# adolfogonzalez3/custom_envs

Measured on AMD Instinct MI355X. Metric: vectorised env-steps/sec, Optimize-v0 @4096 envs, 1/2/4/8 MI355X vs host CPU, higher is better.
Workload: dtype f64; 1 GPU; Optimize-v0 softmax-regression 256x10 (P=20, obs 41), 4096 envs per GPU, B=N=256, 40-step episodes with in-kernel auto-reset, device-resident actions/outputs; envs_per_gpu=4096, global_envs=4096, n_rows=256, n_features=10, n_classes=2, batch_size=256, steps_per_launch=250, outputs=every step kept: a [250]-record slab per launch, parallelism=env-sharded x1 (no collective)

## Files before the change

custom_envs_amd/csrc/optimize_lr_persist.h:

```cpp
#pragma once

#include "optimize_lr_mfma.h"

namespace ce {

struct ManyArgs {
    int k;
    long long act_stride;
    long long out_step;
};

constexpr int kLpWaves = 4;
constexpr int kLpMaxTpw = 8;

#ifndef CE_LP_G4
#define CE_LP_G4 1
#endif
#ifndef CE_LP_G4_XF
#define CE_LP_G4_XF 1
#endif
#ifndef CE_LP_EPI_SLEEP
#define CE_LP_EPI_SLEEP 0
#endif
#ifndef CE_LP_ROW_PRIO
#define CE_LP_ROW_PRIO 3
#endif
#ifndef CE_LP_LOG_HEAD
#define CE_LP_LOG_HEAD 1
#endif
#ifndef CE_LP_WD_HANDOVER
#define CE_LP_WD_HANDOVER 1
#endif
#ifndef CE_LP_GA_REGS
#define CE_LP_GA_REGS 4
#endif
__host__ __device__ constexpr bool lp_g4(int nkf) { return CE_LP_G4 && nkf <= 3; }
constexpr int kLpWdWave = 2;
constexpr int kLpWdRing = 2;

__host__ __device__ constexpr int lp_tpw(int N, int W = kLpWaves) {
    const int per = ((N + 15) / 16 + W - 1) / W;
    return per <= 1 ? 1 : per <= 2 ? 2 : per <= 4 ? 4 : per <= 8 ? 8 : 0;
}
__host__ __device__ constexpr bool lp_pad(int N, int W = kLpWaves) {
    return N % 16 != 0 || (N + 15) / 16 != W * lp_tpw(N, W);
}

#ifdef CE_DIAG
#define LP_STAMP(k)                                                   \
    do {                                                              \
        __builtin_amdgcn_sched_barrier(0);                            \
        lp_st[k] = __builtin_amdgcn_s_memrealtime();                  \
        __builtin_amdgcn_sched_barrier(0);                            \
    } while (0)
#else
#define LP_STAMP(k) \
    do {            \
    } while (0)
#endif

template <int NKF, int TPW, bool PAD, int W>
__global__ __launch_bounds__(kWave * W) void optimize_lr_persist_kernel(StepArgs<double> a, ManyArgs m) {
    constexpr int BLK = kWave * W;
    constexpr int P_MAX = 2 * kLrMaxF;
    constexpr int TD = lr_tile_doubles(NKF);
    constexpr int PR = (kLrEnvs * P_MAX + BLK - 1) / BLK;
    constexpr int OSM = 2 * P_MAX + 4;
    constexpr int NG = TPW < 4 ? TPW : 4;
    __shared__ double red_s[2][W][4][kWave];
    __shared__ double red_l[2][W][kLrEnvs];
    __shared__ double red_h[2][W][kLrEnvs];
    __shared__ __attribute__((aligned(16))) float obs_s[2][kLrEnvs * OSM];
    __shared__ double tab_s[CE_LR_TEXP ? kLrExpTab : 1];

#ifdef CE_DIAG
    unsigned long long lp_st[8] = {0};
#endif
    LP_STAMP(0);
    const int tid = threadIdx.x;
    const int lane = tid & (kWave - 1);
    const int wave = __builtin_amdgcn_readfirstlane(tid >> 6);
    const int c = lane & 15, h = lane >> 4;
    const int E = a.E, F = a.F, P = 2 * F, N = a.N, B = a.B;
    const int OS = a.obs_stride, OL = a.obs_lo;
    const int e0 = blockIdx.x * kLrEnvs;
    const int e = e0 + c;
    const bool env_ok = e < E;
    const unsigned pbase = static_cast<unsigned>(env_ok ? e : 0) * P;
    const double *img = reinterpret_cast<const double *>(a.data);
    const int ntiles = (N + 15) / 16;

#if CE_LR_TEXP
    LrExpSlice<BLK> tslice;
    tslice.load(img + static_cast<unsigned>(ntiles) * TD + kLrMaxF, tid);
#endif
    unsigned ioff[NKF];
    double2 wv[NKF], w0v[NKF];
    float2 av[NKF];
#if CE_LR_NOCLAMP
    double xm[NKF];
    const double *colmax = img + static_cast<unsigned>(ntiles) * TD;
#endif
#pragma unroll
    for (int k = 0; k < NKF; ++k) {
        const int f = 4 * k + h;
        ioff[k] = pbase + (f < F ? 2 * f : 0);
        wv[k] = *reinterpret_cast<const double2 *>(a.W + ioff[k]);
        w0v[k] = *reinterpret_cast<const double2 *>(a.W0 + ioff[k]);
        av[k] = *reinterpret_cast<const float2 *>(a.act + ioff[k]);
#if CE_LR_NOCLAMP
        xm[k] = colmax[f];
#endif
    }
    double xf[TPW][NKF], xg[TPW][4];
    unsigned vmask = 0;
#pragma unroll
    for (int i = 0; i < TPW; ++i) {
        const int t = wave + W * i;
        const bool live = !PAD || t < ntiles;
        const double *ti = img + static_cast<unsigned>(live ? t : 0) * TD;
#pragma unroll
        for (int k = 0; k < NKF; ++k) xf[i][k] = live ? ti[k * kWave + lane] : 0.0;
#pragma unroll
        for (int q = 0; q < 4; ++q) xg[i][q] = live ? ti[(NKF + q) * kWave + lane] : 0.0;
        if constexpr (PAD) {
            const int2 ya = reinterpret_cast<const int2 *>(ti + (NKF + 4) * kWave)[lane];
            const int2 yb = reinterpret_cast<const int2 *>(ti + (NKF + 5) * kWave)[lane];
            const int ys[4] = {ya.x, ya.y, yb.x, yb.y};
#pragma unroll
            for (int q = 0; q < 4; ++q) vmask |= (live && ys[q] >= 0 ? 1u : 0u) << (4 * i + q);
        }
    }
    int step_c = a.step[env_ok ? e : 0];
    const int np_ = kLrEnvs * P;
    const int pmul = (65536 + P - 1) / P;
    int pj[PR], pp[PR], step_p[PR];
    bool prole[PR];
    unsigned gi[PR];
    double g_prev[PR], rG[PR];
#pragma unroll
    for (int r = 0; r < PR; ++r) {
        const int i = tid + r * BLK;
        pj[r] = (i * pmul) >> 16;
        pp[r] = i - pj[r] * P;
        prole[r] = i < np_ && e0 + pj[r] < E;
        gi[r] = static_cast<unsigned>(prole[r] ? e0 + pj[r] : 0) * P + (prole[r] ? pp[r] : 0);
        g_prev[r] = a.G[gi[r]];
        step_p[r] = a.step[prole[r] ? e0 + pj[r] : 0];
    }
    const int sj = tid - (BLK - kLrEnvs);
    const bool srole = sj >= 0 && e0 + sj < E;
    const unsigned es = srole ? e0 + sj : 0;
    double lprev = a.L[es];
    int step_s = a.step[es];
#if CE_LR_TEXP
    tslice.store(tab_s, tid);
    __syncthreads();
#endif
    const double dB = static_cast<double>(B), rB = a.inv_B;
    double rL = rcp_newton2(lprev + 0.1);
#pragma unroll
    for (int r = 0; r < PR; ++r) rG[r] = rcp_newton2(fabs(g_prev[r]) + 1.0);
    if (OL == 0)
        for (int i = tid; i < kLrEnvs * OS; i += BLK) {
            const int j = i / OS, p = i - j * OS;
            if (p < P) obs_s[0][i] = obs_s[1][i] = 0.0f;
        }

    double wd[NKF];
    auto margins = [&]() {
#pragma unroll
        for (int k = 0; k < NKF; ++k) {
            const int f = 4 * k + h;
            const double w0 = wv[k].x - static_cast<double>(av[k].x);
            const double w1 = wv[k].y - static_cast<double>(av[k].y);
            wv[k] = double2{w0, w1};
            wd[k] = f < F ? w0 - w1 : 0.0;
        }
    };
    margins();
#ifdef CE_DIAG
    asm volatile("s_waitcnt vmcnt(0)" ::: "memory");
#endif
    LP_STAMP(1);

    constexpr int QC = 4;
    auto forward = [&](const double (&xv)[NKF]) {
        lr_d4 u = {0.0, 0.0, 0.0, 0.0};
#pragma unroll
        for (int k = 0; k < NKF; ++k) u = __builtin_amdgcn_mfma_f64_16x16x4f64(xv[k], wd[k], u, 0, 0, 0);
        return u;
    };
    const int nenv = E - e0 < kLrEnvs ? E - e0 : kLrEnvs;
    auto flush_obs = [&](int t) {
        float *ob = reinterpret_cast<float *>(reinterpret_cast<char *>(a.obs) + t * m.out_step) +
                    static_cast<unsigned>(e0) * OS;
        const float *src = obs_s[t & 1];
        const int nfl = nenv * OS, n4 = nfl >> 2;
        for (int i = tid; i < n4; i += BLK) {
            typedef float lp_f4 __attribute__((ext_vector_type(4)));
            const lp_f4 v = *reinterpret_cast<const lp_f4 *>(&src[4 * i]);
            asm volatile("global_store_dwordx4 %0, %1, off sc1" ::"v"(ob + 4 * i), "v"(v) : "memory");
        }
        for (int i = 4 * n4 + tid; i < nfl; i += BLK) lr_store(&ob[i], src[i]);
    };

    for (int t = 0; t < m.k; ++t) {
        const int buf = t & 1;
        float2 an[NKF];
        {
            const float *actn = a.act + (t + 1 < m.k ? (t + 1) * m.act_stride : 0);
#pragma unroll
            for (int k = 0; k < NKF; ++k) an[k] = *reinterpret_cast<const float2 *>(actn + ioff[k]);
        }
#if CE_LR_NOCLAMP
        double ub = 0.0;
#pragma unroll
        for (int k = 0; k < NKF; ++k) ub = fma(fabs(wd[k]), xm[k], ub);
        const int tier = lr_tier(ub);
#else
        const int tier = kLrClamped;
#endif
        lr_d4 sacc = {0.0, 0.0, 0.0, 0.0};
        double prod = 1.0, nlog = 0.0, umin = 1.0;
        unsigned miss = 0;
        auto rows = [&](auto tier_c) {
            constexpr int TIER = decltype(tier_c)::value;
#pragma unroll
            for (int g0 = 0; g0 < TPW; g0 += NG) {
                if (g0 > 0) {
                    nlog -= lr_log(prod, tab_s);
                    prod = 1.0;
                }
                lr_d4 u[NG];
#pragma unroll
                for (int i = 0; i < NG; ++i) u[i] = forward(xf[g0 + i]);
#pragma unroll
                for (int i = 0; i < NG; ++i) {
                    double qv[4];
                    static_assert(QC == 4, "the tile's four values go through the exp together");
                    double tx[QC];
                    bool valid[QC];
#pragma unroll
                    for (int j = 0; j < QC; ++j) {
                        if constexpr (TIER == kLrClamped) tx[j] = clamp_u(u[i][j]);
                        else tx[j] = u[i][j];
                        valid[j] = !PAD || ((vmask >> (4 * (g0 + i) + j)) & 1u);
                    }
                    lr_exp_neg<QC>(tx, tab_s);
                    if constexpr (TIER == kLrBatched) {
                        lr_post4(u[i], tx, valid, qv, prod, miss);
                    } else {
#pragma unroll
                        for (int j = 0; j < QC; ++j) lr_post(u[i][j], tx[j], valid[j], qv[j], prod, miss);
                    }
                    lr_tie4<TIER>(u[i], valid, umin);
#pragma unroll
                    for (int q = 0; q < 4; ++q)
                        sacc = __builtin_amdgcn_mfma_f64_16x16x4f64(xg[g0 + i][q], qv[q], sacc, 0, 0, 0);
                }
            }
        };
        lr_run_tier(tier, rows);
        int hits = 4 * TPW - lr_miss_count(miss);
        if (__any(umin < 0x1p-52)) {
#pragma unroll
            for (int i = 0; i < TPW; ++i) {
                const int tt = wave + W * i;
                if (tt >= ntiles) continue;
                const double *ti = img + static_cast<unsigned>(tt) * TD;
                const int2 ya = reinterpret_cast<const int2 *>(ti + (NKF + 4) * kWave)[lane];
                const int2 yb = reinterpret_cast<const int2 *>(ti + (NKF + 5) * kWave)[lane];
                const int yv[4] = {ya.x, ya.y, yb.x, yb.y};
                const lr_d4 uu = forward(xf[i]);
                double tx[4];
#pragma unroll
                for (int q = 0; q < 4; ++q) tx[q] = abs_clamp750(uu[q]);
                exp_neg_multi_clamped<4>(tx);
#pragma unroll
                for (int q = 0; q < 4; ++q)
                    if (yv[q] >= 0 && tx[q] == 1.0) hits += (yv[q] == 0 ? 1 : 0) - lr_hit(uu[q]);
            }
        }
        double lsum = nlog - lr_log(prod, tab_s);
        lsum = fold_pair<16>(lsum, lsum);
        lsum = fold_pair<32>(lsum, lsum);
        const double hsum = static_cast<double>(fold_env_lanes(hits));
#pragma unroll
        for (int r = 0; r < 4; ++r) red_s[buf][wave][r][lane] = sacc[r];
        if (lane < kLrEnvs) {
            red_l[buf][wave][lane] = lsum;
            red_h[buf][wave][lane] = hsum;
        }
        {
            const bool wipe = step_c + 1 >= a.max_steps && a.auto_reset;
            step_c = wipe ? 0 : step_c + 1;
#pragma unroll
            for (int k = 0; k < NKF; ++k)
                if (wipe) wv[k] = w0v[k];
            if (t + 1 < m.k) {
#pragma unroll
                for (int k = 0; k < NKF; ++k) av[k] = an[k];
                margins();
            }
        }
        __syncthreads();
#ifdef CE_DIAG
        if (t == 0) LP_STAMP(2);
        if (t == 1) LP_STAMP(3);
        if (t == m.k - 1) LP_STAMP(4);
#endif
        if (t > 0) flush_obs(t - 1);

        const long long ro = t * m.out_step;
        if (srole) {
            double lt = 0.0, ht = 0.0;
#pragma unroll
            for (int w = 0; w < W; ++w) {
                lt += red_l[buf][w][sj];
                ht += red_h[buf][w][sj];
            }
            const double loss = div_rcp(lt, dB, rB);
            const double acc = div_rcp(ht, dB, rB);
            const double lnew = div_rcp(loss - lprev, lprev + 0.1, rL);
            const int cur = step_s + 1;
            const bool wipe = cur >= a.max_steps && a.auto_reset;
            if (a.reward) lr_store(reinterpret_cast<float *>(reinterpret_cast<char *>(a.reward) + ro) + es,
                                   static_cast<float>(-loss));
            lr_store(reinterpret_cast<float *>(reinterpret_cast<char *>(a.objective) + ro) + es,
                     static_cast<float>(loss));
            lr_store(reinterpret_cast<float *>(reinterpret_cast<char *>(a.accuracy) + ro) + es,
                     static_cast<float>(acc));
            if (a.done) (reinterpret_cast<uint8_t *>(a.done) + ro)[es] = cur >= a.max_steps ? 1 : 0;
            lr_store(reinterpret_cast<int32_t *>(reinterpret_cast<char *>(a.episode_len) + ro) + es, cur);
            obs_s[buf][sj * OS + P - OL] = wipe ? 0.0f : static_cast<float>(lnew);
            lprev = wipe ? 0.0 : lnew;
            step_s = wipe ? 0 : cur;
            rL = rcp_newton2(lprev + 0.1);
        }
#pragma unroll
        for (int r = 0; r < PR; ++r) {
            if (!prole[r]) continue;
            const bool wipe = step_p[r] + 1 >= a.max_steps && a.auto_reset;
            const int f = pp[r] >> 1;
            double sf = 0.0;
#pragma unroll
            for (int w = 0; w < W; ++w) sf += red_s[buf][w][f >> 2][pj[r] + 16 * (f & 3)];
            const double g = div_rcp((pp[r] & 1) ? sf : -sf, dB, rB);
            const double gnew = div_rcp(g, fabs(g_prev[r]) + 1.0, rG[r]);
            obs_s[buf][pj[r] * OS + P + 1 + pp[r] - OL] = wipe ? 0.0f : static_cast<float>(gnew);
            g_prev[r] = wipe ? 0.0 : gnew;
            step_p[r] = wipe ? 0 : step_p[r] + 1;
            rG[r] = rcp_newton2(fabs(g_prev[r]) + 1.0);
        }
    }
    LP_STAMP(5);
    __syncthreads();
    if (m.k > 0) flush_obs(m.k - 1);
    if (wave == 0 && env_ok) {
#pragma unroll
        for (int k = 0; k < NKF; ++k)
            if (4 * k + h < F) {
                lr_store(a.W + ioff[k], wv[k].x);
                lr_store(a.W + ioff[k] + 1, wv[k].y);
            }
    }
#pragma unroll
    for (int r = 0; r < PR; ++r)
        if (prole[r]) lr_store(&a.G[gi[r]], g_prev[r]);
    if (srole) {
        lr_store(&a.L[es], lprev);
        lr_store(&a.step[es], step_s);
    }
#ifdef CE_DIAG
    asm volatile("s_waitcnt vmcnt(0)" ::: "memory");
    LP_STAMP(6);
    const int row = blockIdx.x * W + wave;
    if (row < E && lane < 8) a.diag[static_cast<size_t>(row) * 8 + lane] = lp_st[lane];
#endif
}


template <int NKF, int TPW, bool PAD>
__global__ __launch_bounds__(512) void optimize_lr_persist_ws_kernel(
    double *Wp, const float *actp, const unsigned char *datap, double *Gp, int32_t *stepp, double *Lp,
    unsigned efp, int Np, StepArgs<double> a, ManyArgs m) {
    constexpr int W = 4;
    constexpr int BLK = 512;
    constexpr int EB = BLK - kWave * W;
    constexpr int P_MAX = 2 * kLrMaxF;
    constexpr int TD = lr_tile_doubles(NKF);
    constexpr int PR = (kLrEnvs * P_MAX + EB - 1) / EB;
    constexpr int OSM = 2 * P_MAX + 4;
    constexpr int NG = TPW < 4 ? TPW : 4;
    __shared__ double red_s[2][W][4][kWave];
    __shared__ double red_l[2][W][kLrEnvs];
    __shared__ double red_h[2][W][kLrEnvs];
    __shared__ __attribute__((aligned(16))) float obs_s[2][kLrEnvs * OSM];
    constexpr bool G4 = lp_g4(NKF);
    constexpr int G4S = 14;
    constexpr int NR = CE_LP_GA_REGS < TPW ? CE_LP_GA_REGS : TPW;
    constexpr int GS0 = G4 && NR > 0 ? 1 - NR : -NR;
    constexpr int NGS = TPW + GS0 > 0 ? TPW + GS0 : 1;
    __shared__ __attribute__((aligned(16))) double xgs[G4 ? 1 : W][G4 ? 1 : NGS][4][kWave];
    __shared__ __attribute__((aligned(16))) double xga[G4 ? W : 1][G4 ? NGS : 1][16][G4S];
    __shared__ double tab_s[CE_LR_TEXP ? kLrExpTab : 1];
#if CE_LP_WD_HANDOVER
    __shared__ double wd_s[kLpWdRing][NKF][kWave];
    __shared__ int tier_s[kLpWdRing];
#endif

#ifdef CE_DIAG
    unsigned long long lp_st[8] = {0};
#endif
    LP_STAMP(0);
    const int tid = threadIdx.x;
    const int lane = tid & (kWave - 1);
    const int wave = __builtin_amdgcn_readfirstlane(tid >> 6);
    const int c = lane & 15, h = lane >> 4;
    const int E = static_cast<int>(efp & 0xffffffu), F = static_cast<int>(efp >> 24), P = 2 * F, N = Np, B = a.B;
    const int OS = a.obs_stride, OL = a.obs_lo;
    const int e0 = blockIdx.x * kLrEnvs;
    const double *img = reinterpret_cast<const double *>(datap);
    const int ntiles = (N + 15) / 16;
    const int nenv = E - e0 < kLrEnvs ? E - e0 : kLrEnvs;

#if CE_LR_TEXP
    LrExpSlice<BLK> tslice;
    tslice.load(img + static_cast<unsigned>(ntiles) * TD + kLrMaxF, tid);
#endif
    if (wave < W) {
#if CE_LP_ROW_PRIO > 0
        __builtin_amdgcn_s_setprio(CE_LP_ROW_PRIO);
#endif
#if !CE_LP_WD_HANDOVER
        const int e = e0 + c;
        const bool env_ok = e < E;
        const unsigned pbase = static_cast<unsigned>(env_ok ? e : 0) * P;
        unsigned ioff[NKF];
        double2 wv[NKF], w0v[NKF];
        float2 av[NKF];
#if CE_LR_NOCLAMP
        double xm[NKF];
        const double *colmax = img + static_cast<unsigned>(ntiles) * TD;
#endif
#pragma unroll
        for (int k = 0; k < NKF; ++k) {
            const int f = 4 * k + h;
            ioff[k] = pbase + (f < F ? 2 * f : 0);
            wv[k] = *reinterpret_cast<const double2 *>(Wp + ioff[k]);
            av[k] = *reinterpret_cast<const float2 *>(actp + ioff[k]);
#if CE_LR_NOCLAMP
            xm[k] = colmax[f];
#endif
        }
#endif
        double xf[TPW][NKF];
#if !CE_LP_WD_HANDOVER
#pragma unroll
        for (int k = 0; k < NKF; ++k) w0v[k] = *reinterpret_cast<const double2 *>(a.W0 + ioff[k]);
#endif
        [[maybe_unused]] double gvr[NR > 0 ? NR : 1][G4 ? 4 * NKF : 4];
        unsigned vmask = 0;
#pragma unroll
        for (int i = 0; i < TPW; ++i) {
            const int t = wave + W * i;
            const bool live = !PAD || t < ntiles;
            const double *ti = img + static_cast<unsigned>(live ? t : 0) * TD;
#pragma unroll
            for (int k = 0; k < NKF; ++k) xf[i][k] = live ? ti[k * kWave + lane] : 0.0;
            if constexpr (G4) {
                const int s = i < NR ? 0 : i + GS0;
#if CE_LP_G4_XF
                const int km = 4 * (c & 3) + h, j4 = c >> 2;
#pragma unroll
                for (int g = 0; g < NKF; ++g)
                    if (i >= NR) xga[wave][s][km][j4 * NKF + g] = xf[i][g];
#else
                const int b4 = (lane >> 2) & 3, km = 4 * (lane >> 4) + (lane & 3);
#pragma unroll
                for (int q = 0; q < 4; ++q)
                    if (i >= NR && b4 < NKF) xga[wave][s][km][q * NKF + b4] = live ? ti[(NKF + q) * kWave + lane] : 0.0;
#endif
            } else if (i >= NR) {
#pragma unroll
                for (int q = 0; q < 4; ++q)
                    xgs[wave][i + GS0][q][lane] = live ? ti[(NKF + q) * kWave + lane] : 0.0;
            } else {
#pragma unroll
                for (int q = 0; q < 4; ++q) gvr[i][q] = live ? ti[(NKF + q) * kWave + lane] : 0.0;
            }
            if constexpr (PAD) {
                const int2 ya = reinterpret_cast<const int2 *>(ti + (NKF + 4) * kWave)[lane];
                const int2 yb = reinterpret_cast<const int2 *>(ti + (NKF + 5) * kWave)[lane];
                const int ys[4] = {ya.x, ya.y, yb.x, yb.y};
#pragma unroll
                for (int q = 0; q < 4; ++q) vmask |= (live && ys[q] >= 0 ? 1u : 0u) << (4 * i + q);
            }
        }
        if constexpr (G4 && NR > 0) {
            typedef double lp_d2 __attribute__((ext_vector_type(2)));
            const lp_d2 *src = reinterpret_cast<const lp_d2 *>(&xga[wave][0][4 * (lane >> 4) + (lane & 3)][0]);
#pragma unroll
            for (int i = 0; i < NR; ++i) {
#if CE_LP_G4_XF
                const int km = 4 * (c & 3) + h, j4 = c >> 2;
#pragma unroll
                for (int g = 0; g < NKF; ++g) xga[wave][0][km][j4 * NKF + g] = xf[i][g];
#else
                const int t = wave + W * i;
                const bool live = !PAD || t < ntiles;
                const double *ti = img + static_cast<unsigned>(live ? t : 0) * TD;
                const int b4 = (lane >> 2) & 3, km = 4 * (lane >> 4) + (lane & 3);
#pragma unroll
                for (int q = 0; q < 4; ++q)
                    if (b4 < NKF) xga[wave][0][km][q * NKF + b4] = live ? ti[(NKF + q) * kWave + lane] : 0.0;
#endif
                __builtin_amdgcn_wave_barrier();
#pragma unroll
                for (int p2 = 0; p2 < 2 * NKF; ++p2) {
                    const lp_d2 v = src[p2];
                    gvr[i][2 * p2] = v.x;
                    gvr[i][2 * p2 + 1] = v.y;
                }
                __builtin_amdgcn_wave_barrier();
            }
        }
#if !CE_LP_WD_HANDOVER
        int step_c = stepp[env_ok ? e : 0];
#endif
#if CE_LR_TEXP
        tslice.store(tab_s, tid);
#endif
#if CE_LR_TEXP || CE_LP_WD_HANDOVER
        __syncthreads();
#endif
        double wd[NKF];
#if CE_LP_WD_HANDOVER
        int slot = 0;
#else
        auto margins = [&]() {
#pragma unroll
            for (int k = 0; k < NKF; ++k) {
                const int f = 4 * k + h;
                const double w0 = wv[k].x - static_cast<double>(av[k].x);
                const double w1 = wv[k].y - static_cast<double>(av[k].y);
                wv[k] = double2{w0, w1};
                wd[k] = f < F ? w0 - w1 : 0.0;
            }
        };
        margins();
#endif
#ifdef CE_DIAG
        asm volatile("s_waitcnt vmcnt(0)" ::: "memory");
#endif
        LP_STAMP(1);
        constexpr int QC = 4;
        auto forward = [&](const double (&xv)[NKF]) {
            lr_d4 u = {0.0, 0.0, 0.0, 0.0};
#pragma unroll
            for (int k = 0; k < NKF; ++k) u = __builtin_amdgcn_mfma_f64_16x16x4f64(xv[k], wd[k], u, 0, 0, 0);
            return u;
        };
        for (int t = 0; t < m.k; ++t) {
            const int buf = t & 1;
#if CE_LP_WD_HANDOVER
#pragma unroll
            for (int k = 0; k < NKF; ++k) wd[k] = wd_s[slot][k][lane];
#if CE_LR_NOCLAMP
            const int tier = __builtin_amdgcn_readfirstlane(tier_s[slot]);
#else
            const int tier = kLrClamped;
#endif
            slot = slot == kLpWdRing - 1 ? 0 : slot + 1;
#else
            float2 an[NKF];
            {
                const float *actn = actp + (t + 1 < m.k ? (t + 1) * m.act_stride : 0);
#pragma unroll
                for (int k = 0; k < NKF; ++k) an[k] = *reinterpret_cast<const float2 *>(actn + ioff[k]);
            }
#if CE_LR_NOCLAMP
            double ub = 0.0;
#pragma unroll
            for (int k = 0; k < NKF; ++k) ub = fma(fabs(wd[k]), xm[k], ub);
            const int tier = lr_tier(ub);
#else
            const int tier = kLrClamped;
#endif
#endif
            lr_d4 sacc = {0.0, 0.0, 0.0, 0.0};
            double gacc[NKF];
#pragma unroll
            for (int g = 0; g < NKF; ++g) gacc[g] = 0.0;
            double prod = 1.0, nlog = 0.0, umin = 1.0;
            unsigned miss = 0;
            [[maybe_unused]] LrLogHead lhead = {};
            auto rows = [&](auto tier_c) {
                constexpr int TIER = decltype(tier_c)::value;
#pragma unroll
                for (int g0 = 0; g0 < TPW; g0 += NG) {
                    if (g0 > 0) {
                        nlog -= lr_log(prod, tab_s);
                        prod = 1.0;
                    }
                    lr_d4 u[NG];
#pragma unroll
                    for (int i = 0; i < NG; ++i) u[i] = forward(xf[g0 + i]);
#pragma unroll
                    for (int i = 0; i < NG; ++i) {
                        double gv[G4 ? 4 * NKF : 4];
                        if (g0 + i < NR) {
#pragma unroll
                            for (int j = 0; j < (G4 ? 4 * NKF : 4); ++j) gv[j] = gvr[g0 + i < NR ? g0 + i : 0][j];
                        } else if constexpr (G4) {
                            typedef double lp_d2 __attribute__((ext_vector_type(2)));
                            const lp_d2 *src = reinterpret_cast<const lp_d2 *>(
                                &xga[wave][g0 + i + GS0][4 * (lane >> 4) + (lane & 3)][0]);
#pragma unroll
                            for (int p2 = 0; p2 < 2 * NKF; ++p2) {
                                const lp_d2 v = src[p2];
                                gv[2 * p2] = v.x;
                                gv[2 * p2 + 1] = v.y;
                            }
                        } else {
#pragma unroll
                            for (int q = 0; q < 4; ++q) gv[q] = xgs[wave][g0 + i + GS0][q][lane];
                        }
                        double qv[4];
                        static_assert(QC == 4, "the tile's four values go through the exp together");
                        double tx[QC];
                        bool valid[QC];
#pragma unroll
                        for (int j = 0; j < QC; ++j) {
                            if constexpr (TIER == kLrClamped) tx[j] = clamp_u(u[i][j]);
                            else tx[j] = u[i][j];
                            valid[j] = !PAD || ((vmask >> (4 * (g0 + i) + j)) & 1u);
                        }
                        lr_exp_neg<QC>(tx, tab_s);
                        if constexpr (TIER == kLrBatched) {
                            lr_post4(u[i], tx, valid, qv, prod, miss);
                        } else {
#pragma unroll
                            for (int j = 0; j < QC; ++j)
                                lr_post(u[i][j], tx[j], valid[j], qv[j], prod, miss);
                        }
                        lr_tie4<TIER>(u[i], valid, umin);
#if CE_LP_LOG_HEAD
                        if (g0 + NG >= TPW && i == NG - 1) {
                            lhead = lr_log_head(prod, tab_s);
                            __builtin_amdgcn_sched_barrier(0);
                        }
#endif
                        if constexpr (G4) {
#pragma unroll
                            for (int q = 0; q < 4; ++q)
#pragma unroll
                                for (int g = 0; g < NKF; ++g)
                                    gacc[g] = __builtin_amdgcn_mfma_f64_4x4x4f64(gv[q * NKF + g], qv[q], gacc[g], 0, 0, 0);
                        } else {
#pragma unroll
                            for (int q = 0; q < 4; ++q)
                                sacc = __builtin_amdgcn_mfma_f64_16x16x4f64(gv[q], qv[q], sacc, 0, 0, 0);
                        }
                    }
                }
            };
            lr_run_tier(tier, rows);
            int hits = 4 * TPW - lr_miss_count(miss);
            if (__any(umin < 0x1p-52)) {
#pragma unroll
                for (int i = 0; i < TPW; ++i) {
                    const int tt = wave + W * i;
                    if (tt >= ntiles) continue;
                    const double *ti = img + static_cast<unsigned>(tt) * TD;
                    const int2 ya = reinterpret_cast<const int2 *>(ti + (NKF + 4) * kWave)[lane];
                    const int2 yb = reinterpret_cast<const int2 *>(ti + (NKF + 5) * kWave)[lane];
                    const int yv[4] = {ya.x, ya.y, yb.x, yb.y};
                    const lr_d4 uu = forward(xf[i]);
                    double tx[4];
#pragma unroll
                    for (int q = 0; q < 4; ++q) tx[q] = abs_clamp750(uu[q]);
                    exp_neg_multi_clamped<4>(tx);
#pragma unroll
                    for (int q = 0; q < 4; ++q)
                        if (yv[q] >= 0 && tx[q] == 1.0) hits += (yv[q] == 0 ? 1 : 0) - lr_hit(uu[q]);
                }
            }
#if CE_LP_LOG_HEAD
            double lsum = nlog - lr_log_tail(lhead);
#else
            double lsum = nlog - lr_log(prod, tab_s);
#endif
            lsum = fold_pair<16>(lsum, lsum);
            lsum = fold_pair<32>(lsum, lsum);
            const double hsum = static_cast<double>(fold_env_lanes(hits));
            if constexpr (G4) {
#pragma unroll
                for (int g = 0; g < NKF; ++g) red_s[buf][wave][g][lane] = gacc[g];
            } else {
#pragma unroll
                for (int r = 0; r < 4; ++r) red_s[buf][wave][r][lane] = sacc[r];
            }
            if (lane < kLrEnvs) {
                red_l[buf][wave][lane] = lsum;
                red_h[buf][wave][lane] = hsum;
            }
#if !CE_LP_WD_HANDOVER
            {
                const bool wipe = step_c + 1 >= a.max_steps && a.auto_reset;
                step_c = wipe ? 0 : step_c + 1;
                if (__any(wipe)) {
#pragma unroll
                    for (int k = 0; k < NKF; ++k)
                        if (wipe) wv[k] = w0v[k];
                }
                if (t + 1 < m.k) {
#pragma unroll
                    for (int k = 0; k < NKF; ++k) av[k] = an[k];
                    margins();
                }
            }
#endif
#ifdef CE_DIAG
            if (t == 1) LP_STAMP(7);
#endif
            __syncthreads();
#ifdef CE_DIAG
            if (t == 0) LP_STAMP(2);
            if (t == 1) LP_STAMP(3);
            if (t == m.k - 1) LP_STAMP(4);
#endif
        }
        LP_STAMP(5);
        __syncthreads();
#if !CE_LP_WD_HANDOVER
        if (wave == 0 && env_ok) {
#pragma unroll
            for (int k = 0; k < NKF; ++k)
                if (4 * k + h < F) {
                    lr_store(Wp + ioff[k], wv[k].x);
                    lr_store(Wp + ioff[k] + 1, wv[k].y);
                }
        }
#endif
    } else {
        const int te = tid - kWave * W;
        const int np_ = kLrEnvs * P;
        const int pmul = (65536 + P - 1) / P;
        int pj[PR], pp[PR], step_p[PR];
        bool prole[PR];
        unsigned gi[PR];
        double g_prev[PR], rG[PR];
#pragma unroll
        for (int r = 0; r < PR; ++r) {
            const int i = te + r * EB;
            pj[r] = (i * pmul) >> 16;
            pp[r] = i - pj[r] * P;
            prole[r] = i < np_ && e0 + pj[r] < E;
            gi[r] = static_cast<unsigned>(prole[r] ? e0 + pj[r] : 0) * P + (prole[r] ? pp[r] : 0);
            g_prev[r] = Gp[gi[r]];
            step_p[r] = stepp[prole[r] ? e0 + pj[r] : 0];
        }
        const int sj = te - (EB - kLrEnvs);
        const bool srole = sj >= 0 && e0 + sj < E;
        const unsigned es = srole ? e0 + sj : 0;
        double lprev = Lp[es];
        int step_s = stepp[es];
#if CE_LP_WD_HANDOVER
        const bool wown = wave == W + kLpWdWave;
        const int e = e0 + c;
        const bool env_ok = e < E;
        unsigned ioff[NKF];
        double2 wv[NKF], w0v[NKF];
        float2 an[NKF];
        [[maybe_unused]] double xm[NKF];
        int step_c = 0;
        auto wd_wipe = [&]() {
            const bool wipe = step_c + 1 >= a.max_steps && a.auto_reset;
            step_c = wipe ? 0 : step_c + 1;
            if (__any(wipe)) {
#pragma unroll
                for (int k = 0; k < NKF; ++k)
                    if (wipe) wv[k] = w0v[k];
            }
        };
        auto wd_emit = [&](int slot, const float2 (&av)[NKF]) {
            double wd[NKF];
#pragma unroll
            for (int k = 0; k < NKF; ++k) {
                const int f = 4 * k + h;
                const double w0 = wv[k].x - static_cast<double>(av[k].x);
                const double w1 = wv[k].y - static_cast<double>(av[k].y);
                wv[k] = double2{w0, w1};
                wd[k] = f < F ? w0 - w1 : 0.0;
            }
#if CE_LR_NOCLAMP
            double ub = 0.0;
#pragma unroll
            for (int k = 0; k < NKF; ++k) ub = fma(fabs(wd[k]), xm[k], ub);
            tier_s[slot] = lr_tier(ub);
#endif
#pragma unroll
            for (int k = 0; k < NKF; ++k) wd_s[slot][k][lane] = wd[k];
        };
        auto act_load = [&](int s, float2 (&av)[NKF]) {
            const float *acts = actp + s * m.act_stride;
#pragma unroll
            for (int k = 0; k < NKF; ++k) av[k] = *reinterpret_cast<const float2 *>(acts + ioff[k]);
        };
        if (wown) {
            const unsigned pbase = static_cast<unsigned>(env_ok ? e : 0) * P;
#if CE_LR_NOCLAMP
            const double *colmax = img + static_cast<unsigned>(ntiles) * TD;
#endif
#pragma unroll
            for (int k = 0; k < NKF; ++k) {
                const int f = 4 * k + h;
                ioff[k] = pbase + (f < F ? 2 * f : 0);
                wv[k] = *reinterpret_cast<const double2 *>(Wp + ioff[k]);
                w0v[k] = *reinterpret_cast<const double2 *>(a.W0 + ioff[k]);
#if CE_LR_NOCLAMP
                xm[k] = colmax[f];
#endif
            }
            step_c = stepp[env_ok ? e : 0];
            float2 a0[kLpWdRing][NKF];
#pragma unroll
            for (int s = 0; s < kLpWdRing; ++s)
                if (s < m.k) act_load(s, a0[s]);
            if (kLpWdRing < m.k) act_load(kLpWdRing, an);
#pragma unroll
            for (int s = 0; s < kLpWdRing; ++s) {
                if (s > 0 && s <= m.k) wd_wipe();
                if (s < m.k) wd_emit(s, a0[s]);
            }
        }
#endif
#if CE_LR_TEXP
        tslice.store(tab_s, tid);
#endif
        const double dB = static_cast<double>(B), rB = a.inv_B;
        double rL = rcp_newton2(lprev + 0.1);
#pragma unroll
        for (int r = 0; r < PR; ++r) rG[r] = rcp_newton2(fabs(g_prev[r]) + 1.0);
#if CE_LR_TEXP || CE_LP_WD_HANDOVER
        __syncthreads();
#endif
        auto flush_obs = [&](int t) {
            float *ob = reinterpret_cast<float *>(reinterpret_cast<char *>(a.obs) + t * m.out_step) +
                        static_cast<unsigned>(e0) * OS;
            const float *src = obs_s[t & 1];
            const int nfl = nenv * OS, n4 = nfl >> 2;
            for (int i = te; i < n4; i += EB) {
                typedef float lp_f4 __attribute__((ext_vector_type(4)));
                const lp_f4 v = *reinterpret_cast<const lp_f4 *>(&src[4 * i]);
                asm volatile("global_store_dwordx4 %0, %1, off sc1" ::"v"(ob + 4 * i), "v"(v) : "memory");
            }
            for (int i = 4 * n4 + te; i < nfl; i += EB) lr_store(&ob[i], src[i]);
        };
        if (OL == 0)
            for (int i = te; i < kLrEnvs * OS; i += EB) {
                const int j = i / OS, p = i - j * OS;
                if (p < P) obs_s[0][i] = obs_s[1][i] = 0.0f;
            }
        auto epi_steps = [&](auto pow2_c) {
            auto divB = [&](double x) {
                if constexpr (decltype(pow2_c)::value) return x * rB;
                else return div_rcp(x, dB, rB);
            };
#if CE_LP_WD_HANDOVER
            int wslot = 0;
#endif
            for (int t = 0; t < m.k; ++t) {
                const int buf = t & 1;
                __syncthreads();
#if CE_LP_EPI_SLEEP > 0
                __builtin_amdgcn_s_sleep(CE_LP_EPI_SLEEP);
#endif
    #ifdef CE_DIAG
                if (t == 1) LP_STAMP(2);
    #endif
#if CE_LP_WD_HANDOVER
                if (wown && t + kLpWdRing <= m.k) {
                    wd_wipe();
                    if (t + kLpWdRing < m.k) {
                        float2 av[NKF];
    #pragma unroll
                        for (int k = 0; k < NKF; ++k) av[k] = an[k];
                        if (t + kLpWdRing + 1 < m.k) act_load(t + kLpWdRing + 1, an);
                        wd_emit(wslot, av);
                    }
                }
                wslot = wslot == kLpWdRing - 1 ? 0 : wslot + 1;
#endif
                if (t > 0) flush_obs(t - 1);
                const long long ro = t * m.out_step;
                if (srole) {
                    double lt = 0.0, ht = 0.0;
    #pragma unroll
                    for (int w = 0; w < W; ++w) {
                        lt += red_l[buf][w][sj];
                        ht += red_h[buf][w][sj];
                    }
                    const double loss = divB(lt);
                    const double acc = divB(ht);
                    const double lnew = div_rcp(loss - lprev, lprev + 0.1, rL);
                    const int cur = step_s + 1;
                    const bool wipe = cur >= a.max_steps && a.auto_reset;
                    if (a.reward) lr_store(reinterpret_cast<float *>(reinterpret_cast<char *>(a.reward) + ro) + es,
                                           static_cast<float>(-loss));
                    lr_store(reinterpret_cast<float *>(reinterpret_cast<char *>(a.objective) + ro) + es,
                             static_cast<float>(loss));
                    lr_store(reinterpret_cast<float *>(reinterpret_cast<char *>(a.accuracy) + ro) + es,
                             static_cast<float>(acc));
                    if (a.done) (reinterpret_cast<uint8_t *>(a.done) + ro)[es] = cur >= a.max_steps ? 1 : 0;
                    lr_store(reinterpret_cast<int32_t *>(reinterpret_cast<char *>(a.episode_len) + ro) + es, cur);
                    float ol = static_cast<float>(lnew);
                    lprev = lnew;
                    step_s = cur;
                    if (__any(wipe)) {
                        if (wipe) {
                            ol = 0.0f;
                            lprev = 0.0;
                            step_s = 0;
                        }
                    }
                    obs_s[buf][sj * OS + P - OL] = ol;
                    rL = rcp_newton2(lprev + 0.1);
                }
    #pragma unroll
                for (int r = 0; r < PR; ++r) {
                    if (!prole[r]) continue;
                    const bool wipe = step_p[r] + 1 >= a.max_steps && a.auto_reset;
                    const int f = pp[r] >> 1;
                    double sf = 0.0;
    #pragma unroll
                    for (int w = 0; w < W; ++w) sf += red_s[buf][w][f >> 2][pj[r] + 16 * (f & 3)];
                    const double g = divB((pp[r] & 1) ? sf : -sf);
                    const double gnew = div_rcp(g, fabs(g_prev[r]) + 1.0, rG[r]);
                    float og = static_cast<float>(gnew);
                    g_prev[r] = gnew;
                    step_p[r] = step_p[r] + 1;
                    if (__any(wipe)) {
                        if (wipe) {
                            og = 0.0f;
                            g_prev[r] = 0.0;
                            step_p[r] = 0;
                        }
                    }
                    obs_s[buf][pj[r] * OS + P + 1 + pp[r] - OL] = og;
                    rG[r] = rcp_newton2(fabs(g_prev[r]) + 1.0);
                }
    #ifdef CE_DIAG
                if (t == 1) {
                    asm volatile("s_waitcnt vmcnt(0) lgkmcnt(0)" ::: "memory");
                    LP_STAMP(7);
                }
    #endif
            }
        };
        if ((B & (B - 1)) == 0) epi_steps(std::true_type{});
        else epi_steps(std::false_type{});
        __syncthreads();
        if (m.k > 0) flush_obs(m.k - 1);
#pragma unroll
        for (int r = 0; r < PR; ++r)
            if (prole[r]) lr_store(&Gp[gi[r]], g_prev[r]);
        if (srole) {
            lr_store(&Lp[es], lprev);
            lr_store(&stepp[es], step_s);
        }
#if CE_LP_WD_HANDOVER
        if (wown && env_ok) {
#pragma unroll
            for (int k = 0; k < NKF; ++k)
                if (4 * k + h < F) {
                    lr_store(Wp + ioff[k], wv[k].x);
                    lr_store(Wp + ioff[k] + 1, wv[k].y);
                }
        }
#endif
    }
#ifdef CE_DIAG
    asm volatile("s_waitcnt vmcnt(0)" ::: "memory");
    LP_STAMP(6);
    const int row = blockIdx.x * 8 + wave;
    if (row < E && lane < 8) a.diag[static_cast<size_t>(row) * 8 + lane] = lp_st[lane];
#endif
}

}
```

Measured before the change: 1.916 billion env-steps/s.

## Restructure epilogue waves: shared wipe vote, double-buffered action prefetch, balanced param roles

The epilogue step loop is unrolled by two with compile-time buffer parity. Action loads alternate between two register sets, so the owner wave's prefetch for step t+3 no longer waits on a register copy. The per-role `__any(wipe)` ballots are replaced by one combined vote per step, which guards the wipe branches. Parameter-slot assignment is remapped so the waves without the owner or scalar roles take more slots, and an explicit waitcnt is added before the first barrier. These changes aim to shorten the serial critical path of the epilogue waves, at the cost of more register pressure and code size.

```diff
diff --git a/custom_envs_amd/csrc/optimize_lr_persist.h b/custom_envs_amd/csrc/optimize_lr_persist.h
--- a/custom_envs_amd/csrc/optimize_lr_persist.h
+++ b/custom_envs_amd/csrc/optimize_lr_persist.h
@@ -37,6 +37,24 @@
 __host__ __device__ constexpr bool lp_g4(int nkf) { return CE_LP_G4 && nkf <= 3; }
 constexpr int kLpWdWave = 2;
 constexpr int kLpWdRing = 2;
+#ifndef CE_LP_EPI_WIPE_BRANCH
+#define CE_LP_EPI_WIPE_BRANCH 1
+#endif
+#ifndef CE_LP_EPI_PREFETCH
+#define CE_LP_EPI_PREFETCH 1
+#endif
+#ifndef CE_LP_EPI_LEVEL
+#define CE_LP_EPI_LEVEL 1
+#endif
+template <int PR>
+__device__ inline int lp_param_role(int ew, int lane, int r) {
+#if CE_LP_EPI_LEVEL
+    static_assert(kLpWdWave == 2, "waves 0 and 1 are the ones without the owner or the scalar role");
+    return ew < 2 ? (ew * PR + r) * kWave + lane : (2 * PR + 2 * r + ew - 2) * kWave + lane;
+#else
+    return (4 * r + ew) * kWave + lane;
+#endif
+}
 
 __host__ __device__ constexpr int lp_tpw(int N, int W = kLpWaves) {
     const int per = ((N + 15) / 16 + W - 1) / W;
@@ -57,6 +75,15 @@
 #define LP_STAMP(k) \
     do {            \
     } while (0)
+#endif
+#ifdef CE_LP_ROLE_MARKS
+#define LP_ROLE(s) asm volatile("; lp-role " s)
+#define LP_WIPE_MARK "; lp-role wipe"
+#else
+#define LP_ROLE(s) \
+    do {           \
+    } while (0)
+#define LP_WIPE_MARK ""
 #endif
 
 template <int NKF, int TPW, bool PAD, int W>
@@ -754,7 +781,7 @@
         double g_prev[PR], rG[PR];
 #pragma unroll
         for (int r = 0; r < PR; ++r) {
-            const int i = te + r * EB;
+            const int i = lp_param_role<PR>(wave - W, lane, r);
             pj[r] = (i * pmul) >> 16;
             pp[r] = i - pj[r] * P;
             prole[r] = i < np_ && e0 + pj[r] < E;
@@ -767,23 +794,38 @@
         const unsigned es = srole ? e0 + sj : 0;
         double lprev = Lp[es];
         int step_s = stepp[es];
+        [[maybe_unused]] float2 ana[NKF], anb[NKF];
 #if CE_LP_WD_HANDOVER
         const bool wown = wave == W + kLpWdWave;
         const int e = e0 + c;
         const bool env_ok = e < E;
         unsigned ioff[NKF];
         double2 wv[NKF], w0v[NKF];
-        float2 an[NKF];
         [[maybe_unused]] double xm[NKF];
         int step_c = 0;
-        auto wd_wipe = [&]() {
+        auto wd_vote = [&]() { return __any(step_c + 1 >= a.max_steps && a.auto_reset) != 0; };
+        auto wd_wipe = [&](bool vote) {
             const bool wipe = step_c + 1 >= a.max_steps && a.auto_reset;
+#if CE_LP_EPI_WIPE_BRANCH
+            step_c = step_c + 1;
+            if (vote) {
+#pragma unroll
+                for (int k = 0; k < NKF; ++k) asm volatile("" : "+v"(wv[k].x), "+v"(wv[k].y));
+                asm volatile(LP_WIPE_MARK : "+v"(step_c));
+                if (wipe) {
+                    step_c = 0;
+#pragma unroll
+                    for (int k = 0; k < NKF; ++k) wv[k] = w0v[k];
+                }
+            }
+#else
             step_c = wipe ? 0 : step_c + 1;
             if (__any(wipe)) {
 #pragma unroll
                 for (int k = 0; k < NKF; ++k)
                     if (wipe) wv[k] = w0v[k];
             }
+#endif
         };
         auto wd_emit = [&](int slot, const float2 (&av)[NKF]) {
             double wd[NKF];
@@ -827,12 +869,11 @@
             step_c = stepp[env_ok ? e : 0];
             float2 a0[kLpWdRing][NKF];
 #pragma unroll
-            for (int s = 0; s < kLpWdRing; ++s)
-                if (s < m.k) act_load(s, a0[s]);
-            if (kLpWdRing < m.k) act_load(kLpWdRing, an);
+            for (int s = 0; s < kLpWdRing; ++s) act_load(s < m.k ? s : m.k - 1, a0[s]);
+            act_load(kLpWdRing < m.k ? kLpWdRing : m.k - 1, ana);
 #pragma unroll
             for (int s = 0; s < kLpWdRing; ++s) {
-                if (s > 0 && s <= m.k) wd_wipe();
+                if (s > 0 && s <= m.k) wd_wipe(wd_vote());
                 if (s < m.k) wd_emit(s, a0[s]);
             }
         }
@@ -844,6 +885,7 @@
         double rL = rcp_newton2(lprev + 0.1);
 #pragma unroll
         for (int r = 0; r < PR; ++r) rG[r] = rcp_newton2(fabs(g_prev[r]) + 1.0);
+        __builtin_amdgcn_s_waitcnt(0x0f70);
 #if CE_LR_TEXP || CE_LP_WD_HANDOVER
         __syncthreads();
 #endif
@@ -869,11 +911,8 @@
                 if constexpr (decltype(pow2_c)::value) return x * rB;
                 else return div_rcp(x, dB, rB);
             };
-#if CE_LP_WD_HANDOVER
-            int wslot = 0;
-#endif
-            for (int t = 0; t < m.k; ++t) {
-                const int buf = t & 1;
+            auto epi_step = [&](int t, auto par_c, float2 (&ause)[NKF], float2 (&aload)[NKF]) {
+                const int buf = par_c;
                 __syncthreads();
 #if CE_LP_EPI_SLEEP > 0
                 __builtin_amdgcn_s_sleep(CE_LP_EPI_SLEEP);
@@ -881,22 +920,51 @@
     #ifdef CE_DIAG
                 if (t == 1) LP_STAMP(2);
     #endif
+#if CE_LP_EPI_WIPE_BRANCH
+                bool wany = false;
 #if CE_LP_WD_HANDOVER
-                if (wown && t + kLpWdRing <= m.k) {
-                    wd_wipe();
-                    if (t + kLpWdRing < m.k) {
-                        float2 av[NKF];
+                wany |= wown & (t + kLpWdRing <= m.k) & (step_c + 1 >= a.max_steps);
+#endif
+                wany |= srole & (step_s + 1 >= a.max_steps);
     #pragma unroll
-                        for (int k = 0; k < NKF; ++k) av[k] = an[k];
-                        if (t + kLpWdRing + 1 < m.k) act_load(t + kLpWdRing + 1, an);
-                        wd_emit(wslot, av);
+                for (int r = 0; r < PR; ++r) wany |= prole[r] & (step_p[r] + 1 >= a.max_steps);
+                const bool vote = __any(wany & (a.auto_reset != 0)) != 0;
+#endif
+#if CE_LP_WD_HANDOVER
+                if (wown) {
+                    LP_ROLE("owner begin");
+#if !CE_LP_EPI_WIPE_BRANCH
+                    const bool vote = false;
+#endif
+                    if (t + kLpWdRing <= m.k) {
+                        wd_wipe(vote);
+#if CE_LP_EPI_PREFETCH
+                        if (t + kLpWdRing < m.k) {
+                            act_load(t + kLpWdRing + 1 < m.k ? t + kLpWdRing + 1 : m.k - 1, aload);
+                            wd_emit(buf, ause);
+                        }
+#else
+                        if (t + kLpWdRing < m.k) {
+                            float2 av[NKF];
+    #pragma unroll
+                            for (int k = 0; k < NKF; ++k) av[k] = ause[k];
+                            if (t + kLpWdRing + 1 < m.k) act_load(t + kLpWdRing + 1, aload);
+                            wd_emit(buf, av);
+                        }
+#endif
                     }
-                }
-                wslot = wslot == kLpWdRing - 1 ? 0 : wslot + 1;
-#endif
+    #ifdef CE_DIAG
+                    if (t == 1) LP_STAMP(3);
+    #endif
+                    LP_ROLE("owner end");
+                }
+#endif
+                LP_ROLE("flush begin");
                 if (t > 0) flush_obs(t - 1);
+                LP_ROLE("flush end");
                 const long long ro = t * m.out_step;
                 if (srole) {
+                    LP_ROLE("scalar begin");
                     double lt = 0.0, ht = 0.0;
     #pragma unroll
                     for (int w = 0; w < W; ++w) {
@@ -919,7 +987,12 @@
                     float ol = static_cast<float>(lnew);
                     lprev = lnew;
                     step_s = cur;
+#if CE_LP_EPI_WIPE_BRANCH
+                    if (vote) {
+                        asm volatile(LP_WIPE_MARK : "+v"(ol), "+v"(lprev), "+v"(step_s));
+#else
                     if (__any(wipe)) {
+#endif
                         if (wipe) {
                             ol = 0.0f;
                             lprev = 0.0;
@@ -928,10 +1001,12 @@
                     }
                     obs_s[buf][sj * OS + P - OL] = ol;
                     rL = rcp_newton2(lprev + 0.1);
+                    LP_ROLE("scalar end");
                 }
     #pragma unroll
                 for (int r = 0; r < PR; ++r) {
                     if (!prole[r]) continue;
+                    LP_ROLE("slot begin");
                     const bool wipe = step_p[r] + 1 >= a.max_steps && a.auto_reset;
                     const int f = pp[r] >> 1;
                     double sf = 0.0;
@@ -942,7 +1017,12 @@
                     float og = static_cast<float>(gnew);
                     g_prev[r] = gnew;
                     step_p[r] = step_p[r] + 1;
+#if CE_LP_EPI_WIPE_BRANCH
+                    if (vote) {
+                        asm volatile(LP_WIPE_MARK : "+v"(og), "+v"(g_prev[r]), "+v"(step_p[r]));
+#else
                     if (__any(wipe)) {
+#endif
                         if (wipe) {
                             og = 0.0f;
                             g_prev[r] = 0.0;
@@ -951,14 +1031,26 @@
                     }
                     obs_s[buf][pj[r] * OS + P + 1 + pp[r] - OL] = og;
                     rG[r] = rcp_newton2(fabs(g_prev[r]) + 1.0);
+                    LP_ROLE("slot end");
                 }
     #ifdef CE_DIAG
                 if (t == 1) {
+                    LP_STAMP(4);
                     asm volatile("s_waitcnt vmcnt(0) lgkmcnt(0)" ::: "memory");
                     LP_STAMP(7);
                 }
     #endif
-            }
+            };
+#if CE_LP_EPI_PREFETCH
+            for (int t = 0;; t += 2) {
+                epi_step(t, std::integral_constant<int, 0>{}, ana, anb);
+                if (t + 1 >= m.k) break;
+                epi_step(t + 1, std::integral_constant<int, 1>{}, anb, ana);
+                if (t + 2 >= m.k) break;
+            }
+#else
+            for (int t = 0; t < m.k; ++t) epi_step(t, t & 1, ana, ana);
+#endif
         };
         if ((B & (B - 1)) == 0) epi_steps(std::true_type{});
         else epi_steps(std::false_type{});
```

New measurement: 1.904 billion env-steps/s (median of 2 runs). No clear change (-0.7%).
